# NTT123/vietTTS

Hardware: AMD Instinct MI355X
Metric: audio samples/sec whole-node, HiFi-GAN V1 mel2wave (higher is better)
Workload: dtype bf16; 1 GPU; HiFi-GAN V1 generator, 64 utterances x 1024 mel frames per GPU per step (BASELINE configs[2] shape), bf16; batch_per_gpu=64, frames=1024, parallelism=dp1 utterance-sharded, weights broadcast once, no data-path collective, microbatch=0, streams=0, schedule=engine default: micro-batches of <= 32768 frames on two HIP streams

## Files before the change

viettts_amd/csrc/bf16_common.h:

```cpp
#pragma once

#include <hip/hip_runtime.h>
#include <stdint.h>

#include "vtts_internal.h"

namespace vtts {

typedef __bf16 bf16x8 __attribute__((ext_vector_type(8)));
typedef __bf16 bf16x2 __attribute__((ext_vector_type(2)));
typedef float f32x2 __attribute__((ext_vector_type(2)));
typedef float f32x16 __attribute__((ext_vector_type(16)));
typedef __attribute__((address_space(3))) void* lds_ptr_t;
typedef __attribute__((address_space(1))) const void* glb_ptr_t;

__device__ __forceinline__ unsigned pack_bf16x2(float lo, float hi) {
    f32x2 v = {lo, hi};
    bf16x2 b = __builtin_convertvector(v, bf16x2);
    return __builtin_bit_cast(unsigned, b);
}
__device__ __forceinline__ float bf16_lo(unsigned u) { return __builtin_bit_cast(float, u << 16); }
__device__ __forceinline__ float bf16_hi(unsigned u) { return __builtin_bit_cast(float, u & 0xffff0000u); }
__device__ __forceinline__ void split2(float v0, float v1, unsigned& hi, unsigned& lo) {
    hi = pack_bf16x2(v0, v1);
    lo = pack_bf16x2(v0 - bf16_lo(hi), v1 - bf16_hi(hi));
}
__device__ __forceinline__ void swap_pair(unsigned& pd, unsigned& qd) {
    auto r = __builtin_amdgcn_permlane32_swap(pd, qd, false, false);
    pd = r[0];
    qd = r[1];
}
template <int NMF, int NA, int NB>
__device__ __forceinline__ void pin_loads() {
    int done = 0;
#pragma unroll
    for (int m = 0; m < NMF; ++m) {
        __builtin_amdgcn_sched_group_barrier(0x008, 1, 0);
        const int upto = (m + 1) * (NA + NB) / NMF;
        for (; done < upto; ++done) {
            if (done < NA) __builtin_amdgcn_sched_group_barrier(0x020, 1, 0);
            else __builtin_amdgcn_sched_group_barrier(0x100, 1, 0);
        }
    }
// ... 40 lines not shown
#define VTTS_TL(a, wg, i) do { } while (0)
#define VTTS_TL_ID(a, wg) do { } while (0)
#endif

__device__ __forceinline__ void glds16_asm(const void* gsrc, unsigned lds_dst) {
    unsigned keep;
    asm volatile("s_mov_b32 %0, m0\n\ts_mov_b32 m0, %2\n\ts_nop 0\n\tglobal_load_lds_dwordx4 %1, off\n\ts_mov_b32 m0, %0"
                 : "=&s"(keep)
                 : "v"(gsrc), "s"(lds_dst)
                 : "memory");
}
__device__ __forceinline__ unsigned lds_addr_of(const void* p) {
    return (unsigned)(unsigned long long)(__attribute__((address_space(3))) const void*)p;
}

template <int SPR>
__device__ __forceinline__ int swz_of(int row) {
    constexpr int RPB = SPR >= 16 ? 1 : 16 / SPR;
    constexpr int MASK = (SPR >= 16 ? 16 : SPR) - 1;
    return (row / RPB) & MASK;
}

template <int SPR>
__device__ __forceinline__ int tile_off(int row, int slot) {
    if constexpr (SPR >= 16) return row * (SPR * 16) + ((slot ^ swz_of<SPR>(row)) << 4);
    else return (row >> 4) * (SPR * 256) + (slot << 8) + ((row & 15) << 4);
}
constexpr int tile_rows16(int rows) { return (rows + 15) / 16 * 16; }

}
```

viettts_amd/csrc/engine.hip:

```cpp
#include "../../include/vtts_hifigan.h"

#include <hip/hip_runtime.h>

#include <cmath>
#include <cstdarg>
#include <cstdio>
#include <cstring>
#include <string>
#include <vector>

#include "vtts_internal.h"

using namespace vtts;

namespace {

thread_local std::string g_last_error;

}

int vtts::failf(int code, const char* fmt, ...) {
    char buf[512];
    va_list ap;
    va_start(ap, fmt);
// ... 1096 lines not shown
                    }
                }
                bf16_pack(wc.data(), l.cin, g, reinterpret_cast<unsigned short*>(host.data() + l.off_wb));
                if (l.has_ug) bf16_pack(wc.data(), l.cin, convt_g_pack_geom(l.bcls), reinterpret_cast<unsigned short*>(host.data() + l.off_ug));
            } else {
                bf16_pack(l.w.data(), l.cin, g, reinterpret_cast<unsigned short*>(host.data() + l.off_wb));
                if (l.has_ug) bf16_pack(l.w.data(), l.cin, convt_g_pack_geom(l.bcls), reinterpret_cast<unsigned short*>(host.data() + l.off_ug));
            }
        }
        for (size_t i = 0; i + 1 < h->layers.size(); ++i) {
            const Layer& c1 = h->layers[i];
            if (!c1.has_pair) continue;
            const Layer& c2 = h->layers[i + 1];
            const BPackGeom pg = pair_g_pack_geom(c1.cin, c1.k);
            const size_t half = bf16_packed_bytes(pg);
            bf16_pack(c1.w.data(), c1.cin, pg, reinterpret_cast<unsigned short*>(host.data() + c1.off_pw));
            bf16_pack(c2.w.data(), c2.cin, pg, reinterpret_cast<unsigned short*>(host.data() + c1.off_pw + half));
            float* pb = reinterpret_cast<float*>(host.data() + c1.off_pb);
            memcpy(pb, c1.b.data(), c1.cin * sizeof(float));
            memcpy(pb + c1.cin, c2.b.data(), c1.cin * sizeof(float));
        }
        for (size_t i = 0; i + 5 < h->layers.size(); ++i) {
            const Layer& c0 = h->layers[i];
            if (!c0.has_rb) continue;
            const BPackGeom pg = pair_g_pack_geom(c0.cin, c0.k);
            const size_t one = bf16_packed_bytes(pg);
            float* rb = reinterpret_cast<float*>(host.data() + c0.off_rb);
            for (int q = 0; q < 6; ++q) {
                const Layer& l = h->layers[i + q];
                bf16_pack(l.w.data(), l.cin, pg, reinterpret_cast<unsigned short*>(host.data() + c0.off_rw + q * one));
                memcpy(rb + (size_t)q * c0.cin, l.b.data(), c0.cin * sizeof(float));
            }
// ... 351 lines not shown
```

viettts_amd/csrc/kernels_bf16.hip:

```cpp
#include <hip/hip_runtime.h>
#include <stdint.h>

#include <stdio.h>
#include <string.h>

#include "bf16_common.h"

namespace vtts {

template <int CINP_, int XC_, int CKC_, int COUTP_, int KS_, int MT_, int NT_, int WM_, int WN_, int TG_, int PA_, bool IN_F32_>
struct BTile {
    static constexpr int CINP = CINP_, XC = XC_, CKC = CKC_, COUTP = COUTP_, KS = KS_, MT = MT_, NT = NT_, WM = WM_, WN = WN_;
    static constexpr int TG = TG_, PA = PA_;
    static constexpr bool IN_F32 = IN_F32_;
    static constexpr int THREADS = 64 * WM * WN;
    static constexpr int MR = MT / WM / 32, NR = NT / WN / 32;
    static constexpr int NXC = CINP / XC;
    static constexpr int NCK = XC / CKC;
    static constexpr int SPR = XC / 8;
    static constexpr int P = XC * 2;
    static constexpr int RPB = 16 / SPR;
    static constexpr int ROWS = NT + 2 * PA;
    static constexpr int X_BYTES = ROWS * P;
    static constexpr int KSTEPS = CKC / 16;
// ... 288 lines not shown
        case BCLS_UP1: return mk(256, 64, 1024, 3, 128, 1);
        case BCLS_UP2: return mk(128, 64, 128, 3, 128, 1);
        case BCLS_UP3: return mk(64, 64, 64, 3, 64, 3);
    }
    return mk(0, 0, 0, 0, 0, 0);
}

const char* bf16_kernel_name(int cls, int K) {
    static thread_local char buf[96];
    const BPackGeom g = bf16_pack_geom(cls, K);
    const int xc = g.cinp < 128 ? g.cinp : 128;
    snprintf(buf, sizeof(buf), "conv_bf16_k<BTile<%d, %d, %d, %d, %d,", g.cinp, xc, g.ckc, g.coutp, g.ks);
    return buf;
}

size_t bf16_packed_bytes(const BPackGeom& g) {
    const int ncc = g.cinp / g.ckc, nsl = (g.ks + g.tg - 1) / g.tg;
    return (size_t)(g.coutp / g.mt) * ncc * nsl * ((size_t)g.mt * g.tg * g.ckc * 2);
}

void bf16_pack(const float* Wc, int cin_real, const BPackGeom& g, unsigned short* out) {
    const int ncc = g.cinp / g.ckc, nsl = (g.ks + g.tg - 1) / g.tg, ksteps = g.ckc / 16, mb = g.mt / 32;
    size_t o = 0;
    for (int mtile = 0; mtile < g.coutp / g.mt; ++mtile)
        for (int cc = 0; cc < ncc; ++cc)
            for (int sl = 0; sl < nsl; ++sl)
                for (int tj = 0; tj < g.tg; ++tj)
                    for (int ks = 0; ks < ksteps; ++ks)
                        for (int mblk = 0; mblk < mb; ++mblk)
                            for (int lane = 0; lane < 64; ++lane)
                                for (int e = 0; e < 8; ++e) {
                                    const int j = sl * g.tg + tj;
                                    const int ci = cc * g.ckc + ks * 16 + 8 * (lane >> 5) + e;
                                    const int co = mtile * g.mt + mblk * 32 + (lane & 31);
                                    float w = 0.f;
// ... 74 lines not shown
```

viettts_amd/csrc/kernels_bf16_rbg.hip:

```cpp
#include <stdio.h>
#include <string.h>

#include <type_traits>

#include "bf16_common.h"

namespace vtts {

constexpr int XCD_MAP_MIN_TILES = 192;

template <int C_, int KS_, int N1_, int WM_, int WN_, int PA_, int MINWG_, int XC_ = C_>
struct GTile {
    static constexpr int C = C_, KS = KS_, N1 = N1_, WM = WM_, WN = WN_, PA = PA_, MINWG = MINWG_;
    static constexpr int XC = XC_, NXC = C / XC;
    static constexpr int THREADS = 64 * WM * WN;
    static constexpr int MR = C / WM / 32, NR = N1 / WN / 32;
    static constexpr int H2 = (KS - 1) / 2;
    static constexpr int MAXDIL = 5;
    static constexpr int NT2 = N1 - 2 * H2;
    static constexpr int SPR1 = XC / 8, P1 = XC * 2;
    static constexpr int SPR2 = C / 8, P2 = C * 2;
    static constexpr int ROWSX_MAX = N1 + 2 * H2 * MAXDIL;
    static constexpr int ROWST = N1 + 2 * H2;
    static constexpr int KSTEPS = C / 16;
    static constexpr int KSX = XC / 16;
    static constexpr int NQT = KS * KSTEPS;
    static constexpr int MB = C / 32;
    static constexpr int RA = PA + 1;
    static constexpr bool UNROLL_ALL = (KSX % RA) != 0;
// ... 21 lines not shown
template <class B>
struct GTail : B {
    static constexpr bool TAIL = true;
    static constexpr int TAIL_BYTES = 1024;
    static int lds_bytes(int dil) { return B::tile_bytes(dil) + B::RAW_BYTES + TAIL_BYTES; }
    static_assert(B::RAWRES && B::C == 32 && B::WM == 1, "the tail lives on the C = 32 tile with the LDS-resident residual rows");
    static_assert(B::tile_bytes(B::MAXDIL) + B::RAW_BYTES + TAIL_BYTES <= 80 * 1024, "two workgroups per CU");
};

template <class T>
__global__ __launch_bounds__(T::THREADS, (T::MINWG * T::THREADS + 255) / 256) void resblock_pair_g_bf16_k(BConvArgs a) {
    constexpr int C = T::C, KS = T::KS, N1 = T::N1, WN = T::WN, PA = T::PA, RA = T::RA;
    constexpr int THREADS = T::THREADS, MR = T::MR, NR = T::NR, H2 = T::H2, NT2 = T::NT2;
    constexpr int SPR1 = T::SPR1, P1 = T::P1, SPR2 = T::SPR2, P2 = T::P2, XC = T::XC, NXC = T::NXC, KSX = T::KSX;
    constexpr int KSTEPS = T::KSTEPS, NQT = T::NQT, MB = T::MB, XPT = T::XPT;

    extern __shared__ __attribute__((aligned(16))) unsigned char lds[];
    unsigned char* xt = lds;
    [[maybe_unused]] unsigned char* const xraw = lds + (T::RAWRES ? T::tile_bytes(a.dil) : 0);

    const int tid = threadIdx.x;
    const int lane = tid & 63;
    const int wave = tid >> 6;
    const int wm = wave / WN;
    const int wn = wave % WN;
    const int l31 = lane & 31;
    const int lh = lane >> 5;
    const int b = a.zrev ? (int)(gridDim.z - 1 - blockIdx.z) : (int)blockIdx.z;
    const int Lp = a.L;
    const int L = a.lens ? min(max(a.lens[b], 0) * a.len_mul, a.L) : a.L;
    constexpr int TS = T::TAIL ? NT2 - 2 * T::TAIL_H : NT2;
    const bool xmap = (a.L + TS - 1) / TS >= XCD_MAP_MIN_TILES;
    const int nt = (L + TS - 1) / TS, r = (int)((blockIdx.x + b) & 7), lo = (r * nt) >> 3, hi = ((r + 1) * nt) >> 3;
    const int tile = xmap ? lo + (int)(blockIdx.x >> 3) : (int)blockIdx.x;
    if (xmap && tile >= hi) return;
    const int t0 = tile * TS - (T::TAIL ? T::TAIL_H : 0);
    if (t0 + (T::TAIL ? T::TAIL_H : 0) >= L) return;
    const int dil = a.dil;
    const int h1 = H2 * dil;
    const int rowsx = N1 + 2 * h1;
    const unsigned short* __restrict__ xg = static_cast<const unsigned short*>(a.x) + (size_t)b * Lp * C;
    [[maybe_unused]] const int wg_lin = blockIdx.z * gridDim.x + blockIdx.x;
    VTTS_TL_ID(a, wg_lin);
    VTTS_TL(a, wg_lin, 0);

    f32x16 acc[MR][NR];
    f32x16 bblk[MR];
    auto load_bias = [&](const float* __restrict__ bias) {
        typedef float f32x4 __attribute__((ext_vector_type(4)));
        typedef float f32x8 __attribute__((ext_vector_type(8)));
#pragma unroll
        for (int mr = 0; mr < MR; ++mr) {
            const float* __restrict__ bp = bias + wm * (C / T::WM) + mr * 32 + 4 * lh;
            const f32x4 q0 = *reinterpret_cast<const f32x4*>(bp), q1 = *reinterpret_cast<const f32x4*>(bp + 8);
            const f32x4 q2 = *reinterpret_cast<const f32x4*>(bp + 16), q3 = *reinterpret_cast<const f32x4*>(bp + 24);
            const f32x8 lo = __builtin_shufflevector(q0, q1, 0, 1, 2, 3, 4, 5, 6, 7), hi = __builtin_shufflevector(q2, q3, 0, 1, 2, 3, 4, 5, 6, 7);
            bblk[mr] = __builtin_shufflevector(lo, hi, 0, 1, 2, 3, 4, 5, 6, 7, 8, 9, 10, 11, 12, 13, 14, 15);
        }
    };
    load_bias(a.bias);
    if constexpr (T::TAIL) {
        float* tw = reinterpret_cast<float*>(lds + T::tile_bytes(dil) + T::RAW_BYTES);
        for (int i = tid; i < T::TAIL_KS * C; i += THREADS) tw[i] = a.tail_wf[i];
    }

// ... 6 lines not shown
            for (int q = 0; q < NQT; ++q)
#pragma unroll
                for (int mr = 0; mr < MR; ++mr) aw[q][mr] = __builtin_bit_cast(bf16x8, ap[(size_t)(q * MB + mr) * 64]);
        }
    };
    load_w_all(static_cast<const unsigned char*>(a.wp));

    auto stage_x = [&](int xc, auto xb_tag) {
        constexpr int XB = decltype(xb_tag)::value;
        constexpr int RPI = THREADS / SPR1;
        static_assert(THREADS % SPR1 == 0 && RPI % 16 == 0, "a thread's units share their column and their swizzle");
        const int tx0 = t0 - H2 - h1;
        constexpr int RW = 64 / SPR1;
        const int row0 = SPR1 >= 16 ? tid / SPR1 : wave * RW + lane % RW, c = SPR1 >= 16 ? tid % SPR1 : lane / RW;
        auto act2 = [](unsigned u) { return lrelu01_pack(bf16_lo(u), bf16_hi(u)); };
        unsigned char* const lds0 = xt + tile_off<SPR1>(row0, c);
        [[maybe_unused]] auto keep_raw = [&](int r, int cc, const uint4& raw, bool live) {
            const int rr = r - H2 - h1;
            if (live && rr >= 0 && rr < N1) *reinterpret_cast<uint4*>(xraw + tile_off<SPR1>(rr, cc)) = raw;
        };
        if (tx0 >= 0 && tx0 + XPT * RPI <= L) {
            const unsigned short* __restrict__ g0 = xg + (size_t)(tx0 + row0) * C + xc * XC + c * 8;
#pragma unroll
            for (int i0 = 0; i0 < XPT; i0 += XB) {
                uint4 v[XB];
#pragma unroll
                for (int i = 0; i < XB; ++i)
                    if (i0 + i < XPT) v[i] = *reinterpret_cast<const uint4*>(g0 + (size_t)(i0 + i) * RPI * C);
#if VTTS_TIMELINE
                if (i0 == 0) {
                    VTTS_TL(a, wg_lin, 7);
                    __builtin_amdgcn_s_waitcnt(0x0f70);
                    VTTS_TL(a, wg_lin, 8);
                }
// ... 50 lines not shown
        constexpr int SPRB = decltype(sprb_tag)::value, PB = SPRB * 16, NKS = decltype(nks_tag)::value;
        constexpr bool FRESH = decltype(fresh_tag)::value;
        constexpr int NSTEPS = KS * NKS;
        const uint4* __restrict__ aptr = reinterpret_cast<const uint4*>(wconv) + ((size_t)ks0 * MB + wm * MR) * 64 + lane;
        bf16x8 af[RA][MR], bf[2][NR];
        auto load_a = [&](int tap, int ks, int slot) {
            const int tc = tap < KS ? tap : KS - 1;
#pragma unroll
            for (int mr = 0; mr < MR; ++mr)
                af[slot][mr] = __builtin_bit_cast(bf16x8, aptr[(size_t)((tc * KSTEPS + ks) * MB + mr) * 64]);
        };
        auto load_b = [&](int tap, int ks, int par) {
#pragma unroll
            for (int nr = 0; nr < NR; ++nr) {
                const int row = rowbase0 + tap * dl + nr * 32;
                bf[par][nr] = *reinterpret_cast<const bf16x8*>(xt + tile_off<SPRB>(row, ks * 2 + lh));
            }
        };
        auto mfma_step = [&](int slot, int par, bool first) {
#pragma unroll
            for (int mr = 0; mr < MR; ++mr)
#pragma unroll
                for (int nr = 0; nr < NR; ++nr) {
                    acc[mr][nr] = __builtin_amdgcn_mfma_f32_32x32x16_bf16(af[slot][mr], bf[par][nr], first ? bblk[mr] : acc[mr][nr], 0, 0, 0);

                }
        };
        auto pin_step = [&](bool has_b) {
            constexpr int NM = MR * NR;
            const int mem = MR + (has_b ? NR : 0);
            int done = 0;
// ... 30 lines not shown
                const int sc = sa < NSTEPS ? sa : NSTEPS - 1;
                const int tap = sc / NKS, ks = sc - tap * NKS;
                const int soff = ((tap * KSTEPS + ks0 + ks) * MB) * 1024;
#pragma unroll
                for (int mr = 0; mr < MR; ++mr) {
                    const u32x4_t v = __builtin_amdgcn_raw_buffer_load_b128(rs_w, a_voff + mr * 1024, soff, 0);
                    af[slot][mr] = __builtin_bit_cast(bf16x8, v);
                }
            };
            auto tap_terms = [&](int tap, unsigned& tapaddr, unsigned& xs) {
                const int row = rowbase0 + tap * dl;
                if constexpr (SPRB >= 16) {
                    tapaddr = (unsigned)row * PB;
                    xs = (unsigned)(swz_of<SPRB>(row) ^ lh) << 4;
                } else {
                    tapaddr = (unsigned)tile_off<SPRB>(row, lh);
                    xs = 0;
                }
            };
            auto load_b2 = [&](unsigned tapaddr, unsigned xs, int ks, int par) {
                const unsigned addr = SPRB >= 16 ? tapaddr + (xs ^ (unsigned)(ks << 5)) : tapaddr + (unsigned)(ks << 9);
#pragma unroll
                for (int nr = 0; nr < NR; ++nr) bf[par][nr] = *reinterpret_cast<const bf16x8*>(xt + addr + nr * 32 * PB);
            };
            auto block = [&](int s0, auto first_tag) {
                const int tap = s0 / NKS, ksb = s0 - tap * NKS;
                unsigned ta, xs, tn, xn;
                tap_terms(tap, ta, xs);
                const bool wrap = ksb + UB >= NKS;
                const int tapn = tap + 1 < KS ? tap + 1 : KS - 1;
                tap_terms(wrap ? tapn : tap, tn, xn);
// ... 7 lines not shown
                    pin_step(true);
                }
            };
            block(0, std::integral_constant<bool, FRESH>{});
#pragma nounroll
            for (int s0 = UB; s0 < NSTEPS; s0 += UB) block(s0, std::false_type{});
        }
    };

    auto conv_phase_wreg = [&](int dl, auto sprb_tag) {
        constexpr int SPRB = decltype(sprb_tag)::value;
        bf16x8 bf[2][NR];
        auto load_b = [&](int q, int par) {
            const int tap = q / KSTEPS, ks = q % KSTEPS;
#pragma unroll
            for (int nr = 0; nr < NR; ++nr) bf[par][nr] = *reinterpret_cast<const bf16x8*>(xt + tile_off<SPRB>(rowbase0 + tap * dl + nr * 32, ks * 2 + lh));
        };
        load_b(0, 0);
        __builtin_amdgcn_sched_group_barrier(0x100, NR, 0);
#pragma unroll
        for (int q = 0; q < NQT; ++q) {
            if (q + 1 < NQT) load_b(q + 1, (q + 1) & 1);
#pragma unroll
            for (int mr = 0; mr < MR; ++mr)
#pragma unroll
                for (int nr = 0; nr < NR; ++nr)
                    acc[mr][nr] = __builtin_amdgcn_mfma_f32_32x32x16_bf16(aw[q < NQW ? q : 0][mr], bf[q & 1][nr], q == 0 ? bblk[mr] : acc[mr][nr], 0, 0, 0);
            for (int i = 0; i < MR * NR; ++i) {
                __builtin_amdgcn_sched_group_barrier(0x008, 1, 0);
                if (q + 1 < NQT && i < NR) __builtin_amdgcn_sched_group_barrier(0x100, 1, 0);
            }
        }
    };

#pragma unroll
    for (int xc = 0; xc < NXC; ++xc) {
        if (xc > 0) {
            __syncthreads();
            stage_x(xc, std::integral_constant<int, 4>{});
            __syncthreads();
        }
        if constexpr (T::WREG)
            conv_phase_wreg(dil, std::integral_constant<int, SPR1>{});
        else if (xc == 0)
            conv_phase(static_cast<const unsigned char*>(a.wp), dil, std::integral_constant<int, SPR1>{}, std::integral_constant<int, KSX>{}, 0, std::true_type{});
        else
            conv_phase(static_cast<const unsigned char*>(a.wp), dil, std::integral_constant<int, SPR1>{}, std::integral_constant<int, KSX>{}, xc * KSX, std::false_type{});
    }
    VTTS_TL(a, wg_lin, 2);
    load_w_all(static_cast<const unsigned char*>(a.wp) + T::CONV_BYTES);
    __syncthreads();


    load_bias(a.bias + C);
    {
#pragma unroll
        for (int mr = 0; mr < MR; ++mr) {
#pragma unroll
            for (int p = 0; p < 2; ++p) {
                const int cb = wm * (C / T::WM) + mr * 32 + 16 * p;
#pragma unroll
                for (int nr = 0; nr < NR; ++nr) {
                    const int row = wn * (N1 / WN) + nr * 32 + l31;
                    const int tt = t0 - H2 + row;
                    const bool ok = tt >= 0 && tt < L;
                    const int r0 = 8 * p;
                    unsigned p0 = lrelu01_pack(acc[mr][nr][r0 + 0], acc[mr][nr][r0 + 1]);
                    unsigned p1 = lrelu01_pack(acc[mr][nr][r0 + 2], acc[mr][nr][r0 + 3]);
                    unsigned q0 = lrelu01_pack(acc[mr][nr][r0 + 4], acc[mr][nr][r0 + 5]);
                    unsigned q1 = lrelu01_pack(acc[mr][nr][r0 + 6], acc[mr][nr][r0 + 7]);
                    if (!ok) p0 = p1 = q0 = q1 = 0u;
                    swap_pair(p0, q0);
                    swap_pair(p1, q1);
                    const int slot = (cb >> 3) + lh;
                    *reinterpret_cast<uint4*>(xt + tile_off<SPR2>(row, slot)) = make_uint4(p0, p1, q0, q1);
                }
            }
        }
        for (int u = tid; u < 2 * H2 * SPR2; u += THREADS) {
            const int row = N1 + u % (2 * H2), c = u / (2 * H2);
            *reinterpret_cast<uint4*>(xt + tile_off<SPR2>(row, c)) = make_uint4(0u, 0u, 0u, 0u);
        }
    }
    __syncthreads();
    VTTS_TL(a, wg_lin, 3);

    if constexpr (T::WREG)
        conv_phase_wreg(1, std::integral_constant<int, SPR2>{});
    else
        conv_phase(static_cast<const unsigned char*>(a.wp) + T::CONV_BYTES, 1, std::integral_constant<int, SPR2>{}, std::integral_constant<int, KSTEPS>{}, 0, std::true_type{});
    VTTS_TL(a, wg_lin, 4);

    {
        const float s_out = a.slope_out;
        const float dv = a.div;
        const float rdv = mrf_recip(dv);
        unsigned short* __restrict__ yg = static_cast<unsigned short*>(a.y) + (size_t)b * Lp * C;
        auto add_rows = [&](const unsigned short* __restrict__ src) {
            uint4 rv[MR][2][NR];
#pragma unroll
            for (int mr = 0; mr < MR; ++mr)
#pragma unroll
                for (int p = 0; p < 2; ++p)
#pragma unroll
                    for (int nr = 0; nr < NR; ++nr) {
                        const int t = t0 + wn * (N1 / WN) + nr * 32 + l31;
                        const int tc = t < 0 ? 0 : (t < L ? t : L - 1);
                        rv[mr][p][nr] = *reinterpret_cast<const uint4*>(src + (size_t)tc * C + wm * (C / T::WM) + mr * 32 + 16 * p + 8 * lh);
                    }
#if VTTS_TIMELINE
            VTTS_TL(a, wg_lin, 10);
            __builtin_amdgcn_s_waitcnt(0x0f70);
            VTTS_TL(a, wg_lin, 11);
// ... 1 lines not shown
#pragma unroll
            for (int mr = 0; mr < MR; ++mr)
#pragma unroll
                for (int p = 0; p < 2; ++p)
#pragma unroll
                    for (int nr = 0; nr < NR; ++nr) {
                        uint4 r = rv[mr][p][nr];
                        swap_pair(r.x, r.z);
                        swap_pair(r.y, r.w);
                        const int r0 = 8 * p;
                        acc[mr][nr][r0 + 0] = vadd_raw(bf16_lo(r.x), acc[mr][nr][r0 + 0]); acc[mr][nr][r0 + 1] = vadd_raw(bf16_hi(r.x), acc[mr][nr][r0 + 1]);
                        acc[mr][nr][r0 + 2] = vadd_raw(bf16_lo(r.y), acc[mr][nr][r0 + 2]); acc[mr][nr][r0 + 3] = vadd_raw(bf16_hi(r.y), acc[mr][nr][r0 + 3]);
                        acc[mr][nr][r0 + 4] = vadd_raw(bf16_lo(r.z), acc[mr][nr][r0 + 4]); acc[mr][nr][r0 + 5] = vadd_raw(bf16_hi(r.z), acc[mr][nr][r0 + 5]);
                        acc[mr][nr][r0 + 6] = vadd_raw(bf16_lo(r.w), acc[mr][nr][r0 + 6]); acc[mr][nr][r0 + 7] = vadd_raw(bf16_hi(r.w), acc[mr][nr][r0 + 7]);
                    }
        };
        if constexpr (T::RAWRES) {
#pragma unroll
            for (int mr = 0; mr < MR; ++mr)
#pragma unroll
                for (int p = 0; p < 2; ++p)
#pragma unroll
                    for (int nr = 0; nr < NR; ++nr) {
                        const int col = wn * (N1 / WN) + nr * 32 + l31;
                        uint4 r = *reinterpret_cast<const uint4*>(xraw + tile_off<SPR1>(col, (wm * (C / T::WM) + mr * 32 + 16 * p) / 8 + lh));
                        swap_pair(r.x, r.z);
                        swap_pair(r.y, r.w);
                        const int r0 = 8 * p;
                        acc[mr][nr][r0 + 0] = vadd_raw(bf16_lo(r.x), acc[mr][nr][r0 + 0]); acc[mr][nr][r0 + 1] = vadd_raw(bf16_hi(r.x), acc[mr][nr][r0 + 1]);
                        acc[mr][nr][r0 + 2] = vadd_raw(bf16_lo(r.y), acc[mr][nr][r0 + 2]); acc[mr][nr][r0 + 3] = vadd_raw(bf16_hi(r.y), acc[mr][nr][r0 + 3]);
                        acc[mr][nr][r0 + 4] = vadd_raw(bf16_lo(r.z), acc[mr][nr][r0 + 4]); acc[mr][nr][r0 + 5] = vadd_raw(bf16_hi(r.z), acc[mr][nr][r0 + 5]);
                        acc[mr][nr][r0 + 6] = vadd_raw(bf16_lo(r.w), acc[mr][nr][r0 + 6]); acc[mr][nr][r0 + 7] = vadd_raw(bf16_hi(r.w), acc[mr][nr][r0 + 7]);
                    }
        } else {
            add_rows(xg);
        }
        if (a.acc_add != 0) add_rows(yg);
        VTTS_TL(a, wg_lin, 12);
#pragma unroll
        for (int mr = 0; mr < MR; ++mr) {
#pragma unroll
            for (int p = 0; p < 2; ++p) {
                const int cb = wm * (C / T::WM) + mr * 32 + 16 * p;
#pragma unroll
                for (int nr = 0; nr < NR; ++nr) {
                    const int row = wn * (N1 / WN) + nr * 32 + l31;
                    const int t = t0 + row;
                    const bool ok = row < NT2 && t >= 0 && t < L;
                    float v[8];
#pragma unroll
                    for (int e = 0; e < 8; ++e) v[e] = acc[mr][nr][8 * p + e];
                    if (dv != 1.0f) {
#pragma unroll
                        for (int e = 0; e < 8; ++e) v[e] = v[e] * rdv;
                    }
                    if (s_out != 1.0f) {
#pragma unroll
                        for (int e = 0; e < 8; ++e) v[e] = lrelu_f(v[e], s_out);
                    }
                    unsigned p0 = pack_bf16x2(v[0], v[1]), p1 = pack_bf16x2(v[2], v[3]);
                    unsigned q0 = pack_bf16x2(v[4], v[5]), q1 = pack_bf16x2(v[6], v[7]);
                    swap_pair(p0, q0);
                    swap_pair(p1, q1);
                    if constexpr (T::TAIL) {
                        const uint4 o = ok ? make_uint4(p0, p1, q0, q1) : make_uint4(0u, 0u, 0u, 0u);
                        if (row < NT2) *reinterpret_cast<uint4*>(xraw + tile_off<SPR1>(row, (cb >> 3) + lh)) = o;
                    } else {
                        if (ok) *reinterpret_cast<uint4*>(yg + (size_t)t * C + cb + 8 * lh) = make_uint4(p0, p1, q0, q1);
                    }
                }
            }
        }
    }
    if constexpr (T::TAIL) {
        __syncthreads();
        const float* tw = reinterpret_cast<const float*>(lds + T::tile_bytes(dil) + T::RAW_BYTES);
        const float tb = a.tail_bias[0];
        for (int n = tid; n < TS; n += THREADS) {
            const int t = t0 + T::TAIL_H + n;
            if (t >= L) break;
            float accp = 0.f;
#pragma unroll
            for (int j = 0; j < T::TAIL_KS; ++j) {
#pragma unroll
                for (int c = 0; c < SPR1; ++c) {
                    const uint4 v = *reinterpret_cast<const uint4*>(xraw + tile_off<SPR1>(n + j, c));
                    const float* w = tw + j * C + c * 8;
                    accp = fmaf(w[0], bf16_lo(v.x), accp); accp = fmaf(w[1], bf16_hi(v.x), accp);
                    accp = fmaf(w[2], bf16_lo(v.y), accp); accp = fmaf(w[3], bf16_hi(v.y), accp);
                    accp = fmaf(w[4], bf16_lo(v.z), accp); accp = fmaf(w[5], bf16_hi(v.z), accp);
                    accp = fmaf(w[6], bf16_lo(v.w), accp); accp = fmaf(w[7], bf16_hi(v.w), accp);
                }
            }
            a.tail_wav[(size_t)b * Lp + t] = tanhf(accp + tb);
        }
    }
    VTTS_TL(a, wg_lin, 6);
}

#ifndef VTTS_EXP_LDS_PAD
#define VTTS_EXP_LDS_PAD 0
#endif
#ifndef VTTS_G64_N1
#define VTTS_G64_N1 512
#define VTTS_G64_WG 2
#endif
#ifndef VTTS_G32_N1
#define VTTS_G32_N1 512
#define VTTS_G32_WG 2
#endif
#ifndef VTTS_G128K3_N1
#define VTTS_G128K3_N1 256
#define VTTS_G128K3_WG 2
#endif
template <int KS> using G128 = GTile<128, KS, KS == 3 ? VTTS_G128K3_N1 : 256, 2, 2, 3, KS == 3 ? VTTS_G128K3_WG : 2>;
template <int KS> using G64 = GTile<64, KS, VTTS_G64_N1, 1, 4, 3, VTTS_G64_WG>;
#ifndef VTTS_G32_PA
#define VTTS_G32_PA 3
#endif
template <int KS> using G32 = GTile<32, KS, VTTS_G32_N1, 1, 4, VTTS_G32_PA, VTTS_G32_WG>;
template <int KS> using G256 = GTile<256, KS, 128, 4, 1, 3, 2, 128>;
template <int KS> using G256S = GTile<256, KS, 64, 4, 1, 3, 2, 128>;
template <int KS> using G128S = GTile<128, KS, 128, 2, 2, 3, 2>;
template <int KS> using G64S = GTile<64, KS, 256, 1, 4, 3, 2>;
template <int KS> using G32S = GTile<32, KS, 256, 1, 4, 3, 2>;
constexpr long G_MIN_WGS = 384;
template <class T>
static hipError_t launch_g(const BConvArgs& a, hipStream_t s) {
    static DynLdsOnce once;
    if (hipError_t e = set_max_dynamic_lds(reinterpret_cast<const void*>(&resblock_pair_g_bf16_k<T>), T::lds_bytes(T::MAXDIL) + VTTS_EXP_LDS_PAD, once); e != hipSuccess) return e;
    if (a.dil < 1 || a.dil > T::MAXDIL) return hipErrorInvalidValue;
    constexpr int TS = T::TAIL ? T::NT2 - 2 * T::TAIL_H : T::NT2;
    dim3 grid((a.L + TS - 1) / TS, 1, a.B);
    if ((int)grid.x >= XCD_MAP_MIN_TILES) grid.x = (grid.x + 7) / 8 * 8;
    hipLaunchKernelGGL(resblock_pair_g_bf16_k<T>, grid, dim3(T::THREADS), T::lds_bytes(a.dil) + VTTS_EXP_LDS_PAD, s, a);
    return hipGetLastError();
}

// ... 15 lines not shown
        case 64: return narrow(G64<11>::NT2) ? launch_g_ks<G64S>(a, K, s) : launch_g_ks<G64>(a, K, s);
        case 32:
            if (a.tail_wav) {
                if (K != 11) return hipErrorInvalidValue;
                return narrow(G32<11>::NT2) ? launch_g<GTail<G32S<11>>>(a, s) : launch_g<GTail<G32<11>>>(a, s);
            }
            return narrow(G32<11>::NT2) ? launch_g_ks<G32S>(a, K, s) : launch_g_ks<G32>(a, K, s);
    }
    return hipErrorInvalidValue;
}

bool pair_tail_bf16_supported(int C, int K, int post_cin, int post_cout, int post_k) { return C == 32 && K == 11 && post_cin == 32 && post_cout == 1 && post_k == 7; }

BPackGeom pair_g_pack_geom(int C, int K) { return BPackGeom{C, C, C, K, C, 1}; }

const char* pair_g_kernel_name(int C, int K) {
    static thread_local char buf[96];
    snprintf(buf, sizeof(buf), "resblock_pair_g_bf16_k<GTile<%d, %d,", C, K);
    return buf;
}

bool pair_bf16_supported(int C, int K, int dil) {
    return (C == 256 || C == 128 || C == 64 || C == 32) && (K == 3 || K == 7 || K == 11) && dil >= 1 && dil <= 5;
}

}
```

viettts_amd/csrc/vtts_internal.h:

```cpp
#pragma once

#include <hip/hip_runtime.h>
#include <stddef.h>
#include <stdint.h>
#include <string.h>

#include "../../include/vtts_hifigan.h"

#define VTTS_API extern "C" __attribute__((visibility("default")))

namespace vtts {

int failf(int code, const char* fmt, ...);

#define HIP_TRY(expr)                                                                                          \
    do {                                                                                                       \
        hipError_t _e = (expr);                                                                                \
        if (_e != hipSuccess)                                                                                  \
            return vtts::failf(VTTS_ERR_HIP, "%s failed: %s (%s:%d)", #expr, hipGetErrorString(_e), __FILE__, __LINE__); \
    } while (0)

inline size_t align_up(size_t v, size_t a) { return (v + a - 1) / a * a; }

inline int check_blob(const void* dev_blob, size_t bytes, size_t need) {
// ... 126 lines not shown
    int acc_add;
    int tile_pref;
    float div;
    int zrev;
    unsigned long long* dbg;
    float* tail_wav;
    const float* tail_wf;
    const float* tail_bias;
};

struct BPackGeom { int cinp, ckc, coutp, ks, mt, tg; };

hipError_t launch_conv_bf16(int cls, int K, const BConvArgs& a, hipStream_t s);
BPackGeom bf16_pack_geom(int cls, int K);
const char* bf16_kernel_name(int cls, int K);
size_t bf16_packed_bytes(const BPackGeom& g);
void bf16_pack(const float* Wc, int cin_real, const BPackGeom& g, unsigned short* out);
bool pair_bf16_supported(int C, int K, int dil);
bool pair_tail_bf16_supported(int C, int K, int post_cin, int post_cout, int post_k);
hipError_t launch_pair_g_bf16(int C, int K, const BConvArgs& a, hipStream_t s);
BPackGeom pair_g_pack_geom(int C, int K);
const char* pair_g_kernel_name(int C, int K);
bool resblock_bf16_supported(int C, int K, const int* dils);
bool resblock_bf16_preferred(int C, int K);
hipError_t launch_resblock_bf16(int C, int K, const BConvArgs& a, hipStream_t s);
hipError_t launch_convt_g_bf16(int cls, const BConvArgs& a, hipStream_t s);
BPackGeom convt_g_pack_geom(int cls);
hipError_t launch_conv_post_bf16(const BConvArgs& a, float* wav, float* pre_act, hipStream_t s);
hipError_t launch_bf16_to_f32(const void* in, float* out, size_t n, hipStream_t s);
hipError_t launch_f32_to_bf16(const float* in, void* out, size_t n, hipStream_t s);


constexpr int NAT_RES_H = 512, NAT_RES_PN = 256, NAT_RES_MELMAX = 128;
constexpr int NAT_RES_XCH_ELEMS = NAT_RES_MELMAX + 2 * NAT_RES_PN + 2 * NAT_RES_H;
struct NatResidentArgs {
    const float* w1;
// ... 19 lines not shown
```

Measured before the change: 420.3 million samples/s.

## Add 16x16x32 MFMA path for resblock pair conv tiles with C>=128

Adds an alternative path to the fused resblock pair kernel that uses 16x16x32 bf16 MFMA blocks instead of 32x32 blocks for selected channel/kernel-size combinations (C=256 with K=11, C=128 with K=7/11). It brings a matching weight pack layout, a 16-block LDS swizzle, permlane16-based epilogue shuffles, and a software-pipelined A-ring and B double-buffer loop. The aim is better MFMA throughput, register use or scheduling for these layers, at the cost of more code complexity and a second weight packing format.

```diff
diff --git a/viettts_amd/csrc/bf16_common.h b/viettts_amd/csrc/bf16_common.h
--- a/viettts_amd/csrc/bf16_common.h
+++ b/viettts_amd/csrc/bf16_common.h
@@ -27,6 +27,11 @@
 }
 __device__ __forceinline__ void swap_pair(unsigned& pd, unsigned& qd) {
     auto r = __builtin_amdgcn_permlane32_swap(pd, qd, false, false);
+    pd = r[0];
+    qd = r[1];
+}
+__device__ __forceinline__ void swap_pair16(unsigned& pd, unsigned& qd) {
+    auto r = __builtin_amdgcn_permlane16_swap(pd, qd, false, false);
     pd = r[0];
     qd = r[1];
 }
@@ -97,16 +102,20 @@
     return (unsigned)(unsigned long long)(__attribute__((address_space(3))) const void*)p;
 }
 
-template <int SPR>
+template <int SPR, int BLK = 32>
 __device__ __forceinline__ int swz_of(int row) {
+    if constexpr (BLK == 16) {
+        static_assert(SPR >= 16, "the 16-block image is a row-major image");
+        return (row & 7) | ((row & 1) << 3);
+    }
     constexpr int RPB = SPR >= 16 ? 1 : 16 / SPR;
     constexpr int MASK = (SPR >= 16 ? 16 : SPR) - 1;
     return (row / RPB) & MASK;
 }
 
-template <int SPR>
+template <int SPR, int BLK = 32>
 __device__ __forceinline__ int tile_off(int row, int slot) {
-    if constexpr (SPR >= 16) return row * (SPR * 16) + ((slot ^ swz_of<SPR>(row)) << 4);
+    if constexpr (SPR >= 16) return row * (SPR * 16) + ((slot ^ swz_of<SPR, BLK>(row)) << 4);
     else return (row >> 4) * (SPR * 256) + (slot << 8) + ((row & 15) << 4);
 }
 constexpr int tile_rows16(int rows) { return (rows + 15) / 16 * 16; }
diff --git a/viettts_amd/csrc/engine.hip b/viettts_amd/csrc/engine.hip
--- a/viettts_amd/csrc/engine.hip
+++ b/viettts_amd/csrc/engine.hip
@@ -1134,8 +1134,8 @@
             const Layer& c2 = h->layers[i + 1];
             const BPackGeom pg = pair_g_pack_geom(c1.cin, c1.k);
             const size_t half = bf16_packed_bytes(pg);
-            bf16_pack(c1.w.data(), c1.cin, pg, reinterpret_cast<unsigned short*>(host.data() + c1.off_pw));
-            bf16_pack(c2.w.data(), c2.cin, pg, reinterpret_cast<unsigned short*>(host.data() + c1.off_pw + half));
+            pair_g_pack(c1.w.data(), c1.cin, c1.k, reinterpret_cast<unsigned short*>(host.data() + c1.off_pw));
+            pair_g_pack(c2.w.data(), c2.cin, c1.k, reinterpret_cast<unsigned short*>(host.data() + c1.off_pw + half));
             float* pb = reinterpret_cast<float*>(host.data() + c1.off_pb);
             memcpy(pb, c1.b.data(), c1.cin * sizeof(float));
             memcpy(pb + c1.cin, c2.b.data(), c1.cin * sizeof(float));
diff --git a/viettts_amd/csrc/kernels_bf16.hip b/viettts_amd/csrc/kernels_bf16.hip
--- a/viettts_amd/csrc/kernels_bf16.hip
+++ b/viettts_amd/csrc/kernels_bf16.hip
@@ -326,11 +326,6 @@
     return buf;
 }
 
-size_t bf16_packed_bytes(const BPackGeom& g) {
-    const int ncc = g.cinp / g.ckc, nsl = (g.ks + g.tg - 1) / g.tg;
-    return (size_t)(g.coutp / g.mt) * ncc * nsl * ((size_t)g.mt * g.tg * g.ckc * 2);
-}
-
 void bf16_pack(const float* Wc, int cin_real, const BPackGeom& g, unsigned short* out) {
     const int ncc = g.cinp / g.ckc, nsl = (g.ks + g.tg - 1) / g.tg, ksteps = g.ckc / 16, mb = g.mt / 32;
     size_t o = 0;
diff --git a/viettts_amd/csrc/kernels_bf16_rbg.hip b/viettts_amd/csrc/kernels_bf16_rbg.hip
--- a/viettts_amd/csrc/kernels_bf16_rbg.hip
+++ b/viettts_amd/csrc/kernels_bf16_rbg.hip
@@ -2,17 +2,28 @@
 #include <string.h>
 
 #include <type_traits>
+#include <utility>
 
 #include "bf16_common.h"
 
 namespace vtts {
 
+template <class F, int... I>
+__device__ __forceinline__ void static_for(std::integer_sequence<int, I...>, F&& f) {
+    (f(std::integral_constant<int, I>{}), ...);
+}
+
 constexpr int XCD_MAP_MIN_TILES = 192;
 
-template <int C_, int KS_, int N1_, int WM_, int WN_, int PA_, int MINWG_, int XC_ = C_>
+template <int C_, int KS_, int N1_, int WM_, int WN_, int PA_, int MINWG_, int XC_ = C_, int BLK_ = 32>
 struct GTile {
-    static constexpr int C = C_, KS = KS_, N1 = N1_, WM = WM_, WN = WN_, PA = PA_, MINWG = MINWG_;
+    static constexpr int C = C_, KS = KS_, N1 = N1_, WM = WM_, WN = WN_, PA = PA_, MINWG = MINWG_, BLK = BLK_;
     static constexpr int XC = XC_, NXC = C / XC;
+    static constexpr int MR16 = C / WM / 16, NR16 = N1 / WN / 16, NH = NR16 / 4;
+    static constexpr int KS32 = C / 32, KSX32 = XC / 32;
+        static constexpr int LA16 = 3, RA16 = LA16 + 1;
+    static_assert(BLK == 32 || BLK == 16, "MFMA block shape");
+    static_assert(BLK == 32 || (XC >= 128 && C / WM == 64 && (N1 / WN) % 64 == 0 && KSX32 % 4 == 0 && 4 % RA16 == 0), "16-block tiles: C >= 128, 64-row wave tiles");
     static constexpr int THREADS = 64 * WM * WN;
     static constexpr int MR = C / WM / 32, NR = N1 / WN / 32;
     static constexpr int H2 = (KS - 1) / 2;
@@ -64,6 +75,10 @@
     constexpr int THREADS = T::THREADS, MR = T::MR, NR = T::NR, H2 = T::H2, NT2 = T::NT2;
     constexpr int SPR1 = T::SPR1, P1 = T::P1, SPR2 = T::SPR2, P2 = T::P2, XC = T::XC, NXC = T::NXC, KSX = T::KSX;
     constexpr int KSTEPS = T::KSTEPS, NQT = T::NQT, MB = T::MB, XPT = T::XPT;
+    constexpr int BLK = T::BLK;
+    constexpr bool B16 = BLK == 16;
+    constexpr int MR16 = T::MR16, NR16 = T::NR16, NH = T::NH;
+    static_assert(!B16 || (!T::RAWRES && !T::TAIL && !T::WREG && !T::UNROLL_ALL), "16-block tiles are the rolled-loop C >= 128 tiles");
 
     extern __shared__ __attribute__((aligned(16))) unsigned char lds[];
     unsigned char* xt = lds;
@@ -76,6 +91,8 @@
     const int wn = wave % WN;
     const int l31 = lane & 31;
     const int lh = lane >> 5;
+    const int l15 = lane & 15;
+    const int lg = lane >> 4;
     const int b = a.zrev ? (int)(gridDim.z - 1 - blockIdx.z) : (int)blockIdx.z;
     const int Lp = a.L;
     const int L = a.lens ? min(max(a.lens[b], 0) * a.len_mul, a.L) : a.L;
@@ -94,11 +111,18 @@
     VTTS_TL_ID(a, wg_lin);
     VTTS_TL(a, wg_lin, 0);
 
-    f32x16 acc[MR][NR];
-    f32x16 bblk[MR];
+    typedef float f32x4 __attribute__((ext_vector_type(4)));
+    f32x16 acc[B16 ? 1 : MR][B16 ? 1 : NR];
+    f32x16 bblk[B16 ? 1 : MR];
+    f32x4 acc16[B16 ? MR16 : 1][B16 ? NR16 : 1];
+    f32x4 bblk16[B16 ? MR16 : 1];
     auto load_bias = [&](const float* __restrict__ bias) {
-        typedef float f32x4 __attribute__((ext_vector_type(4)));
         typedef float f32x8 __attribute__((ext_vector_type(8)));
+        if constexpr (B16) {
+#pragma unroll
+            for (int mr = 0; mr < MR16; ++mr) bblk16[mr] = *reinterpret_cast<const f32x4*>(bias + wm * (C / T::WM) + mr * 16 + 4 * lg);
+            return;
+        }
 #pragma unroll
         for (int mr = 0; mr < MR; ++mr) {
             const float* __restrict__ bp = bias + wm * (C / T::WM) + mr * 32 + 4 * lh;
@@ -135,10 +159,10 @@
         constexpr int RW = 64 / SPR1;
         const int row0 = SPR1 >= 16 ? tid / SPR1 : wave * RW + lane % RW, c = SPR1 >= 16 ? tid % SPR1 : lane / RW;
         auto act2 = [](unsigned u) { return lrelu01_pack(bf16_lo(u), bf16_hi(u)); };
-        unsigned char* const lds0 = xt + tile_off<SPR1>(row0, c);
+        unsigned char* const lds0 = xt + tile_off<SPR1, BLK>(row0, c);
         [[maybe_unused]] auto keep_raw = [&](int r, int cc, const uint4& raw, bool live) {
             const int rr = r - H2 - h1;
-            if (live && rr >= 0 && rr < N1) *reinterpret_cast<uint4*>(xraw + tile_off<SPR1>(rr, cc)) = raw;
+            if (live && rr >= 0 && rr < N1) *reinterpret_cast<uint4*>(xraw + tile_off<SPR1, BLK>(rr, cc)) = raw;
         };
         if (tx0 >= 0 && tx0 + XPT * RPI <= L) {
             const unsigned short* __restrict__ g0 = xg + (size_t)(tx0 + row0) * C + xc * XC + c * 8;
@@ -219,7 +243,7 @@
 #pragma unroll
             for (int nr = 0; nr < NR; ++nr) {
                 const int row = rowbase0 + tap * dl + nr * 32;
-                bf[par][nr] = *reinterpret_cast<const bf16x8*>(xt + tile_off<SPRB>(row, ks * 2 + lh));
+                bf[par][nr] = *reinterpret_cast<const bf16x8*>(xt + tile_off<SPRB, BLK>(row, ks * 2 + lh));
             }
         };
         auto mfma_step = [&](int slot, int par, bool first) {
@@ -280,7 +304,7 @@
                     tapaddr = (unsigned)row * PB;
                     xs = (unsigned)(swz_of<SPRB>(row) ^ lh) << 4;
                 } else {
-                    tapaddr = (unsigned)tile_off<SPRB>(row, lh);
+                    tapaddr = (unsigned)tile_off<SPRB, BLK>(row, lh);
                     xs = 0;
                 }
             };
@@ -318,7 +342,7 @@
         auto load_b = [&](int q, int par) {
             const int tap = q / KSTEPS, ks = q % KSTEPS;
 #pragma unroll
-            for (int nr = 0; nr < NR; ++nr) bf[par][nr] = *reinterpret_cast<const bf16x8*>(xt + tile_off<SPRB>(rowbase0 + tap * dl + nr * 32, ks * 2 + lh));
+            for (int nr = 0; nr < NR; ++nr) bf[par][nr] = *reinterpret_cast<const bf16x8*>(xt + tile_off<SPRB, BLK>(rowbase0 + tap * dl + nr * 32, ks * 2 + lh));
         };
         load_b(0, 0);
         __builtin_amdgcn_sched_group_barrier(0x100, NR, 0);
@@ -337,6 +361,89 @@
         }
     };
 
+
+    const int rowbase16 = wn * (N1 / WN) + l15;
+    auto conv_phase16 = [&](const unsigned char* __restrict__ wconv, int dl, auto sprb_tag, auto nks_tag, int ks0, auto fresh_tag) {
+        constexpr int SPRB = decltype(sprb_tag)::value, PB = SPRB * 16, NKS = decltype(nks_tag)::value;
+        constexpr bool FRESH = decltype(fresh_tag)::value;
+        constexpr int NSTEPS = KS * NKS, LA = T::LA16, RA = T::RA16, UB = 4, APU = MR16 / NH;
+        static_assert(NKS % UB == 0 && UB % RA == 0 && (UB * NH) % 2 == 0, "ring slot / B parity must be compile-time in the block loop");
+        const auto rs_w = __builtin_amdgcn_make_buffer_rsrc(const_cast<unsigned char*>(wconv), 0, (int)T::CONV_BYTES, 0x00020000);
+        const unsigned a_voff = (unsigned)((wm * MR16) * 64 + lane) * 16;
+        bf16x8 af[RA][MR16], bf[2][4];
+        auto load_a = [&](int sa, auto h_tag, auto slot_tag) {
+            constexpr int h = decltype(h_tag)::value, slot = decltype(slot_tag)::value;
+            const int sc = sa < NSTEPS ? sa : NSTEPS - 1;
+            const int tap = sc / NKS, ks = sc - tap * NKS;
+            const int soff = ((tap * T::KS32 + ks0 + ks) * (C / 16)) * 1024;
+#pragma unroll
+            for (int m = h * APU; m < (h + 1) * APU; ++m) af[slot][m] = __builtin_bit_cast(bf16x8, __builtin_amdgcn_raw_buffer_load_b128(rs_w, a_voff + m * 1024, soff, 0));
+        };
+        auto tap_terms = [&](int tap, unsigned& tapaddr, unsigned& xs) {
+            const int row = rowbase16 + tap * dl;
+            tapaddr = (unsigned)row * PB;
+            xs = (unsigned)(swz_of<SPRB, 16>(row) ^ lg) << 4;
+        };
+        auto load_b = [&](unsigned tapaddr, unsigned xs, int ks, int h, auto par_tag) {
+            const unsigned addr = tapaddr + (xs ^ (unsigned)(ks << 6));
+#pragma unroll
+            for (int nr = 0; nr < 4; ++nr) bf[decltype(par_tag)::value][nr] = *reinterpret_cast<const bf16x8*>(xt + addr + (4 * h + nr) * 16 * PB);
+        };
+        auto pin_unit = [&]() {
+            int done = 0;
+#pragma unroll
+            for (int i = 0; i < 16; ++i) {
+                __builtin_amdgcn_sched_group_barrier(0x008, 1, 0);
+                const int upto = (i + 1) * (4 + APU) / 16;
+#pragma unroll
+                for (; done < upto; ++done) {
+                    if (done < 4) __builtin_amdgcn_sched_group_barrier(0x100, 1, 0);
+                    else __builtin_amdgcn_sched_group_barrier(0x020, 1, 0);
+                }
+            }
+        };
+        unsigned ta0, xs0;
+        tap_terms(0, ta0, xs0);
+        static_for(std::make_integer_sequence<int, LA * NH>{}, [&](auto v) {
+            constexpr int s = decltype(v)::value / NH, h = decltype(v)::value % NH;
+            load_a(s, std::integral_constant<int, h>{}, std::integral_constant<int, s % RA>{});
+        });
+        load_b(ta0, xs0, 0, 0, std::integral_constant<int, 0>{});
+        __builtin_amdgcn_sched_group_barrier(0x020, MR16 * LA, 0);
+        __builtin_amdgcn_sched_group_barrier(0x100, 4, 0);
+        auto block = [&](int s0) {
+            const int tap = s0 / NKS, ksb = s0 - tap * NKS;
+            unsigned ta, xs, tn, xn;
+            tap_terms(tap, ta, xs);
+            const bool wrap = ksb + UB >= NKS;
+            const int tapn = tap + 1 < KS ? tap + 1 : KS - 1;
+            tap_terms(wrap ? tapn : tap, tn, xn);
+            const int ksn = wrap ? 0 : ksb + UB;
+            static_for(std::make_integer_sequence<int, UB * NH>{}, [&](auto v) {
+                constexpr int u = decltype(v)::value, i = u / NH, h = u % NH;
+                load_a(s0 + i + LA, std::integral_constant<int, h>{}, std::integral_constant<int, (i + LA) % RA>{});
+                constexpr auto par = std::integral_constant<int, (u + 1) & 1>{};
+                if constexpr (h + 1 < NH) load_b(ta, xs, ksb + i, h + 1, par);
+                else if constexpr (i + 1 < UB) load_b(ta, xs, ksb + i + 1, 0, par);
+                else load_b(tn, xn, ksn, 0, par);
+#pragma unroll
+                for (int nr = 0; nr < 4; ++nr)
+#pragma unroll
+                    for (int mr = 0; mr < MR16; ++mr)
+                        acc16[mr][4 * h + nr] = __builtin_amdgcn_mfma_f32_16x16x32_bf16(af[i % RA][mr], bf[u & 1][nr], acc16[mr][4 * h + nr], 0, 0, 0);
+                pin_unit();
+            });
+        };
+        if constexpr (FRESH) {
+#pragma unroll
+            for (int mr = 0; mr < MR16; ++mr)
+#pragma unroll
+                for (int nr = 0; nr < NR16; ++nr) acc16[mr][nr] = bblk16[mr];
+        }
+#pragma nounroll
+        for (int s0 = 0; s0 < NSTEPS; s0 += UB) block(s0);
+    };
+
 #pragma unroll
     for (int xc = 0; xc < NXC; ++xc) {
         if (xc > 0) {
@@ -344,7 +451,10 @@
             stage_x(xc, std::integral_constant<int, 4>{});
             __syncthreads();
         }
-        if constexpr (T::WREG)
+        if constexpr (B16) {
+            if (xc == 0) conv_phase16(static_cast<const unsigned char*>(a.wp), dil, std::integral_constant<int, SPR1>{}, std::integral_constant<int, T::KSX32>{}, 0, std::true_type{});
+            else conv_phase16(static_cast<const unsigned char*>(a.wp), dil, std::integral_constant<int, SPR1>{}, std::integral_constant<int, T::KSX32>{}, xc * T::KSX32, std::false_type{});
+        } else if constexpr (T::WREG)
             conv_phase_wreg(dil, std::integral_constant<int, SPR1>{});
         else if (xc == 0)
             conv_phase(static_cast<const unsigned char*>(a.wp), dil, std::integral_constant<int, SPR1>{}, std::integral_constant<int, KSX>{}, 0, std::true_type{});
@@ -357,7 +467,27 @@
 
 
     load_bias(a.bias + C);
+    [[maybe_unused]] const int col16 = wn * (N1 / WN) + 16 * (lg & 1) + l15;
     {
+        if constexpr (B16) {
+#pragma unroll
+            for (int mr = 0; mr < MR16; ++mr) {
+                const int cb = wm * (C / T::WM) + mr * 16;
+#pragma unroll
+                for (int j = 0; j < NR16 / 2; ++j) {
+                    const int tp = t0 - H2 + wn * (N1 / WN) + 32 * j + l15, tq = tp + 16;
+                    unsigned p0 = lrelu01_pack(acc16[mr][2 * j][0], acc16[mr][2 * j][1]);
+                    unsigned p1 = lrelu01_pack(acc16[mr][2 * j][2], acc16[mr][2 * j][3]);
+                    unsigned q0 = lrelu01_pack(acc16[mr][2 * j + 1][0], acc16[mr][2 * j + 1][1]);
+                    unsigned q1 = lrelu01_pack(acc16[mr][2 * j + 1][2], acc16[mr][2 * j + 1][3]);
+                    if (!(tp >= 0 && tp < L)) p0 = p1 = 0u;
+                    if (!(tq >= 0 && tq < L)) q0 = q1 = 0u;
+                    swap_pair16(p0, q0);
+                    swap_pair16(p1, q1);
+                    *reinterpret_cast<uint4*>(xt + tile_off<SPR2, BLK>(col16 + 32 * j, (cb >> 3) + (lg >> 1))) = make_uint4(p0, p1, q0, q1);
+                }
+            }
+        } else {
 #pragma unroll
         for (int mr = 0; mr < MR; ++mr) {
 #pragma unroll
@@ -377,19 +507,22 @@
                     swap_pair(p0, q0);
                     swap_pair(p1, q1);
                     const int slot = (cb >> 3) + lh;
-                    *reinterpret_cast<uint4*>(xt + tile_off<SPR2>(row, slot)) = make_uint4(p0, p1, q0, q1);
-                }
-            }
+                    *reinterpret_cast<uint4*>(xt + tile_off<SPR2, BLK>(row, slot)) = make_uint4(p0, p1, q0, q1);
+                }
+            }
+        }
         }
         for (int u = tid; u < 2 * H2 * SPR2; u += THREADS) {
             const int row = N1 + u % (2 * H2), c = u / (2 * H2);
-            *reinterpret_cast<uint4*>(xt + tile_off<SPR2>(row, c)) = make_uint4(0u, 0u, 0u, 0u);
+            *reinterpret_cast<uint4*>(xt + tile_off<SPR2, BLK>(row, c)) = make_uint4(0u, 0u, 0u, 0u);
         }
     }
     __syncthreads();
     VTTS_TL(a, wg_lin, 3);
 
-    if constexpr (T::WREG)
+    if constexpr (B16)
+        conv_phase16(static_cast<const unsigned char*>(a.wp) + T::CONV_BYTES, 1, std::integral_constant<int, SPR2>{}, std::integral_constant<int, T::KS32>{}, 0, std::true_type{});
+    else if constexpr (T::WREG)
         conv_phase_wreg(1, std::integral_constant<int, SPR2>{});
     else
         conv_phase(static_cast<const unsigned char*>(a.wp) + T::CONV_BYTES, 1, std::integral_constant<int, SPR2>{}, std::integral_constant<int, KSTEPS>{}, 0, std::true_type{});
@@ -401,6 +534,31 @@
         const float rdv = mrf_recip(dv);
         unsigned short* __restrict__ yg = static_cast<unsigned short*>(a.y) + (size_t)b * Lp * C;
         auto add_rows = [&](const unsigned short* __restrict__ src) {
+            if constexpr (B16) {
+                uint4 rv[MR16][NR16 / 2];
+#pragma unroll
+                for (int mr = 0; mr < MR16; ++mr)
+#pragma unroll
+                    for (int j = 0; j < NR16 / 2; ++j) {
+                        const int t = t0 + col16 + 32 * j;
+                        const int tc = t < 0 ? 0 : (t < L ? t : L - 1);
+                        rv[mr][j] = *reinterpret_cast<const uint4*>(src + (size_t)tc * C + wm * (C / T::WM) + mr * 16 + 8 * (lg >> 1));
+                    }
+#pragma unroll
+                for (int mr = 0; mr < MR16; ++mr)
+#pragma unroll
+                    for (int j = 0; j < NR16 / 2; ++j) {
+                        uint4 r = rv[mr][j];
+                        swap_pair16(r.x, r.z);
+                        swap_pair16(r.y, r.w);
+                        f32x4& ap = acc16[mr][2 * j];
+                        f32x4& aq = acc16[mr][2 * j + 1];
+                        ap[0] = vadd_raw(bf16_lo(r.x), ap[0]); ap[1] = vadd_raw(bf16_hi(r.x), ap[1]);
+                        ap[2] = vadd_raw(bf16_lo(r.y), ap[2]); ap[3] = vadd_raw(bf16_hi(r.y), ap[3]);
+                        aq[0] = vadd_raw(bf16_lo(r.z), aq[0]); aq[1] = vadd_raw(bf16_hi(r.z), aq[1]);
+                        aq[2] = vadd_raw(bf16_lo(r.w), aq[2]); aq[3] = vadd_raw(bf16_hi(r.w), aq[3]);
+                    }
+            } else {
             uint4 rv[MR][2][NR];
 #pragma unroll
             for (int mr = 0; mr < MR; ++mr)
@@ -432,6 +590,7 @@
                         acc[mr][nr][r0 + 4] = vadd_raw(bf16_lo(r.z), acc[mr][nr][r0 + 4]); acc[mr][nr][r0 + 5] = vadd_raw(bf16_hi(r.z), acc[mr][nr][r0 + 5]);
                         acc[mr][nr][r0 + 6] = vadd_raw(bf16_lo(r.w), acc[mr][nr][r0 + 6]); acc[mr][nr][r0 + 7] = vadd_raw(bf16_hi(r.w), acc[mr][nr][r0 + 7]);
                     }
+            }
         };
         if constexpr (T::RAWRES) {
 #pragma unroll
@@ -441,7 +600,7 @@
 #pragma unroll
                     for (int nr = 0; nr < NR; ++nr) {
                         const int col = wn * (N1 / WN) + nr * 32 + l31;
-                        uint4 r = *reinterpret_cast<const uint4*>(xraw + tile_off<SPR1>(col, (wm * (C / T::WM) + mr * 32 + 16 * p) / 8 + lh));
+                        uint4 r = *reinterpret_cast<const uint4*>(xraw + tile_off<SPR1, BLK>(col, (wm * (C / T::WM) + mr * 32 + 16 * p) / 8 + lh));
                         swap_pair(r.x, r.z);
                         swap_pair(r.y, r.w);
                         const int r0 = 8 * p;
@@ -455,6 +614,37 @@
         }
         if (a.acc_add != 0) add_rows(yg);
         VTTS_TL(a, wg_lin, 12);
+        if constexpr (B16) {
+#pragma unroll
+            for (int mr = 0; mr < MR16; ++mr) {
+                const int cb = wm * (C / T::WM) + mr * 16;
+#pragma unroll
+                for (int j = 0; j < NR16 / 2; ++j) {
+                    const int row = col16 + 32 * j;
+                    const int t = t0 + row;
+                    const bool ok = row < NT2 && t >= 0 && t < L;
+                    float v[8];
+#pragma unroll
+                    for (int e = 0; e < 4; ++e) {
+                        v[e] = acc16[mr][2 * j][e];
+                        v[4 + e] = acc16[mr][2 * j + 1][e];
+                    }
+                    if (dv != 1.0f) {
+#pragma unroll
+                        for (int e = 0; e < 8; ++e) v[e] = v[e] * rdv;
+                    }
+                    if (s_out != 1.0f) {
+#pragma unroll
+                        for (int e = 0; e < 8; ++e) v[e] = lrelu_f(v[e], s_out);
+                    }
+                    unsigned p0 = pack_bf16x2(v[0], v[1]), p1 = pack_bf16x2(v[2], v[3]);
+                    unsigned q0 = pack_bf16x2(v[4], v[5]), q1 = pack_bf16x2(v[6], v[7]);
+                    swap_pair16(p0, q0);
+                    swap_pair16(p1, q1);
+                    if (ok) *reinterpret_cast<uint4*>(yg + (size_t)t * C + cb + 8 * (lg >> 1)) = make_uint4(p0, p1, q0, q1);
+                }
+            }
+        } else {
 #pragma unroll
         for (int mr = 0; mr < MR; ++mr) {
 #pragma unroll
@@ -482,12 +672,13 @@
                     swap_pair(p1, q1);
                     if constexpr (T::TAIL) {
                         const uint4 o = ok ? make_uint4(p0, p1, q0, q1) : make_uint4(0u, 0u, 0u, 0u);
-                        if (row < NT2) *reinterpret_cast<uint4*>(xraw + tile_off<SPR1>(row, (cb >> 3) + lh)) = o;
+                        if (row < NT2) *reinterpret_cast<uint4*>(xraw + tile_off<SPR1, BLK>(row, (cb >> 3) + lh)) = o;
                     } else {
                         if (ok) *reinterpret_cast<uint4*>(yg + (size_t)t * C + cb + 8 * lh) = make_uint4(p0, p1, q0, q1);
                     }
                 }
             }
+        }
         }
     }
     if constexpr (T::TAIL) {
@@ -502,7 +693,7 @@
             for (int j = 0; j < T::TAIL_KS; ++j) {
 #pragma unroll
                 for (int c = 0; c < SPR1; ++c) {
-                    const uint4 v = *reinterpret_cast<const uint4*>(xraw + tile_off<SPR1>(n + j, c));
+                    const uint4 v = *reinterpret_cast<const uint4*>(xraw + tile_off<SPR1, BLK>(n + j, c));
                     const float* w = tw + j * C + c * 8;
                     accp = fmaf(w[0], bf16_lo(v.x), accp); accp = fmaf(w[1], bf16_hi(v.x), accp);
                     accp = fmaf(w[2], bf16_lo(v.y), accp); accp = fmaf(w[3], bf16_hi(v.y), accp);
@@ -531,15 +722,20 @@
 #define VTTS_G128K3_N1 256
 #define VTTS_G128K3_WG 2
 #endif
-template <int KS> using G128 = GTile<128, KS, KS == 3 ? VTTS_G128K3_N1 : 256, 2, 2, 3, KS == 3 ? VTTS_G128K3_WG : 2>;
+constexpr int g_mfma_blk(int C, int KS) {
+    return C == 256 ? (KS == 3 ? 32 : KS == 7 ? 32 : 16)
+         : C == 128 ? (KS == 3 ? 32 : KS == 7 ? 16 : 16)
+                    : 32;
+}
+template <int KS> using G128 = GTile<128, KS, KS == 3 ? VTTS_G128K3_N1 : 256, 2, 2, 3, KS == 3 ? VTTS_G128K3_WG : 2, 128, g_mfma_blk(128, KS)>;
 template <int KS> using G64 = GTile<64, KS, VTTS_G64_N1, 1, 4, 3, VTTS_G64_WG>;
 #ifndef VTTS_G32_PA
 #define VTTS_G32_PA 3
 #endif
 template <int KS> using G32 = GTile<32, KS, VTTS_G32_N1, 1, 4, VTTS_G32_PA, VTTS_G32_WG>;
-template <int KS> using G256 = GTile<256, KS, 128, 4, 1, 3, 2, 128>;
-template <int KS> using G256S = GTile<256, KS, 64, 4, 1, 3, 2, 128>;
-template <int KS> using G128S = GTile<128, KS, 128, 2, 2, 3, 2>;
+template <int KS> using G256 = GTile<256, KS, 128, 4, 1, 3, 2, 128, g_mfma_blk(256, KS)>;
+template <int KS> using G256S = GTile<256, KS, 64, 4, 1, 3, 2, 128, g_mfma_blk(256, KS)>;
+template <int KS> using G128S = GTile<128, KS, 128, 2, 2, 3, 2, 128, g_mfma_blk(128, KS)>;
 template <int KS> using G64S = GTile<64, KS, 256, 1, 4, 3, 2>;
 template <int KS> using G32S = GTile<32, KS, 256, 1, 4, 3, 2>;
 constexpr long G_MIN_WGS = 384;
@@ -585,6 +781,13 @@
 
 BPackGeom pair_g_pack_geom(int C, int K) { return BPackGeom{C, C, C, K, C, 1}; }
 
+int pair_g_mfma_blk(int C, int K) { return g_mfma_blk(C, K); }
+
+void pair_g_pack(const float* Wc, int C, int K, unsigned short* out) {
+    if (g_mfma_blk(C, K) == 16) pair_g_pack16(Wc, C, K, out);
+    else bf16_pack(Wc, C, pair_g_pack_geom(C, K), out);
+}
+
 const char* pair_g_kernel_name(int C, int K) {
     static thread_local char buf[96];
     snprintf(buf, sizeof(buf), "resblock_pair_g_bf16_k<GTile<%d, %d,", C, K);
diff --git a/viettts_amd/csrc/vtts_internal.h b/viettts_amd/csrc/vtts_internal.h
--- a/viettts_amd/csrc/vtts_internal.h
+++ b/viettts_amd/csrc/vtts_internal.h
@@ -164,12 +164,29 @@
 hipError_t launch_conv_bf16(int cls, int K, const BConvArgs& a, hipStream_t s);
 BPackGeom bf16_pack_geom(int cls, int K);
 const char* bf16_kernel_name(int cls, int K);
-size_t bf16_packed_bytes(const BPackGeom& g);
+inline size_t bf16_packed_bytes(const BPackGeom& g) {
+    const int ncc = g.cinp / g.ckc, nsl = (g.ks + g.tg - 1) / g.tg;
+    return (size_t)(g.coutp / g.mt) * ncc * nsl * ((size_t)g.mt * g.tg * g.ckc * 2);
+}
 void bf16_pack(const float* Wc, int cin_real, const BPackGeom& g, unsigned short* out);
 bool pair_bf16_supported(int C, int K, int dil);
 bool pair_tail_bf16_supported(int C, int K, int post_cin, int post_cout, int post_k);
 hipError_t launch_pair_g_bf16(int C, int K, const BConvArgs& a, hipStream_t s);
 BPackGeom pair_g_pack_geom(int C, int K);
+int pair_g_mfma_blk(int C, int K);
+inline size_t pair_g_pack16_bytes(int C, int K) { return (size_t)K * (C / 32) * (C / 16) * 64 * 8 * sizeof(unsigned short); }
+inline void pair_g_pack16(const float* Wc, int C, int K, unsigned short* out) {
+    size_t o = 0;
+    for (int tap = 0; tap < K; ++tap)
+        for (int ks = 0; ks < C / 32; ++ks)
+            for (int mblk = 0; mblk < C / 16; ++mblk)
+                for (int lane = 0; lane < 64; ++lane)
+                    for (int e = 0; e < 8; ++e) {
+                        const int ci = 32 * ks + 8 * (lane >> 4) + e, co = 16 * mblk + (lane & 15);
+                        out[o++] = f32_to_bf16_rne(Wc[((size_t)tap * C + ci) * C + co]);
+                    }
+}
+void pair_g_pack(const float* Wc, int C, int K, unsigned short* out);
 const char* pair_g_kernel_name(int C, int K);
 bool resblock_bf16_supported(int C, int K, const int* dils);
 bool resblock_bf16_preferred(int C, int K);
```

Measured after the change: 430.0 million samples/s (median of 6 runs). 1.02x the previous value.
